# damlobster/DotsBoxesAZ

Measured on AMD Instinct MI355X. Metric: mcts_node_expansions_per_sec, higher is better.
Workload: dtype f32 via f16x3 (hi,lo)-split MFMA, f32 accumulate; max |dp|,|dv| vs torch fp32 = 1e-6 (tests/test_hip_nn.py)

## Files before the change

dotsboxesaz_amd/csrc/nn.hip:

```cpp
#include <math.h>
#include <stddef.h>
#include <stdlib.h>
#include <string.h>

#include <map>
#include <string>
#include <vector>

#include "nn.h"
#include "tower_perm.h"
#include "tower_plan.h"

typedef float f32x4 __attribute__((ext_vector_type(4)));

#define CONV_THREADS 512

struct TowerArgs;
typedef void (*TowerKernel)(Geo, TowerArgs);
struct TowerLaunch {
    TowerKernel kernel;
    size_t lds;
    int role, S;
    enum Grid { PER_GROUP, ONE_ROUND, ONE_ROUND_AT_MOST } grid;
    bool fallback;
// ... 118 lines not shown
#define F16_GUARD 60000.0f

union u128h { f32x4 f; f16x8 h; };

template <int C, int PREC>
__device__ __forceinline__ void act_store(float *lds, int row, int c, float v, bool &ovf)
{
    if constexpr (PREC == 0) {
        lds[row * (C + 8) + c] = v;
    } else {
        _Float16 *h = reinterpret_cast<_Float16 *>(lds) + (size_t)row * ((C + 8) * 2);
        const float x = v * ACT_SCALE;
        ovf |= fabsf(x) > F16_GUARD;
        const _Float16 hi = (_Float16)x;
        h[c] = hi;
        h[C + c] = (_Float16)(x - (float)hi);
    }
}
template <int C, int PREC>
__device__ __forceinline__ float act_load(const float *lds, int row, int c)
{
    if constexpr (PREC == 0) {
        return lds[row * (C + 8) + c];
    } else {
        const _Float16 *h = reinterpret_cast<const _Float16 *>(lds) + (size_t)row * ((C + 8) * 2);
        return ((float)h[c] + (float)h[C + c]) * (1.0f / ACT_SCALE);
    }
}

__device__ __forceinline__ f32x4 relu4(f32x4 v)
{
    v[0] = fmaxf(v[0], 0.f); v[1] = fmaxf(v[1], 0.f); v[2] = fmaxf(v[2], 0.f); v[3] = fmaxf(v[3], 0.f);
    return v;
}
__device__ __forceinline__ float max4(f32x4 v) { return fmaxf(fmaxf(v[0], v[1]), fmaxf(v[2], v[3])); }

template <int C>
__device__ __forceinline__ void h3_store(_Float16 *ph, bool valid, f32x4 v)
{
    union { f16x2 h[2]; u32x2 u; } oh, ol;
#pragma unroll
    for (int q = 0; q < 2; q++) {
        const f32x2 x = {v[2 * q], v[2 * q + 1]};
        const f16x2 h = __builtin_convertvector(x, f16x2);
        oh.h[q] = h;
        ol.h[q] = __builtin_convertvector(x - __builtin_convertvector(h, f32x2), f16x2);
    }
    if (valid) {
        *reinterpret_cast<u32x2 *>(ph) = oh.u;
        *reinterpret_cast<u32x2 *>(ph + C) = ol.u;
    }
}

#ifdef DBAZ_STAMP
#define STAMP(var)                                                                      \
    do {                                                                                \
        __builtin_amdgcn_sched_barrier(0);                                              \
        asm volatile("s_memtime %0\n\ts_waitcnt lgkmcnt(0)" : "=s"(var)::"memory");     \
        __builtin_amdgcn_sched_barrier(0);                                              \
    } while (0)
#else
#define STAMP(var) do { } while (0)
#endif

struct WPre { f32x4 h0, l0, h1, l1; };

template <int C>
__device__ __forceinline__ void wpre_load(WPre &pre, const f32x4 *wpk_layer, int wave, int lane)
{
    constexpr int N = 9 * (C / 32);
    const f32x4 *wb = wpk_layer + (size_t)(wave & 3) * N * 2 * 64 + lane;
    pre.h0 = wb[0];
    pre.l0 = wb[64];
    pre.h1 = wb[128];
    pre.l1 = wb[192];
}

template <int C, int NTT, bool RR = false>
__device__ __forceinline__ void conv_lds_h3(const f32x4 *__restrict__ src4, f32x4 *dst4, const f32x4 *__restrict__ wpk ,
                                            const float *__restrict__ bias, float oscale, const int *vm, int rowbase,
                                            int zbase, int W, int R, int wave, int lane, int residual, bool &ovf_out, int tbase,
                                            const float *post_s, const float *post_t, WPre &pre, const f32x4 *next_wpk,
                                            f32x4 (&res)[NTT], unsigned long long *stamps = nullptr)
{
    static_assert(!RR || C <= 64, "one cout tile per wave");

    unsigned long long t0 = 0, t1 = 0, t2 = 0, t3 = 0;
    (void)t0; (void)t1; (void)t2; (void)t3; (void)stamps;
    constexpr int S4 = (C + 8) / 4;
    constexpr int KS = C / 32;
    constexpr int LO = C / 8;
    constexpr int N = 9 * KS;
    const int jrow = lane & 15, gq = lane >> 4;
    bool ovf = false;
    for (int ct = wave & 3; ct < C / 16; ct += 4) {
        f32x4 acc[NTT];
#pragma unroll
        for (int t = 0; t < NTT; t++) acc[t] = (f32x4){0.f, 0.f, 0.f, 0.f};
        const f32x4 *wbase = wpk + (size_t)ct * N * 2 * 64 + lane;
        u128h a_h[3], a_l[3];
        u128h bh[NTT], bl[NTT];
        const char *sb = reinterpret_cast<const char *>(src4);
        int ab[NTT];
#pragma unroll
        for (int t = 0; t < NTT; t++)
            ab[t] = ((vm[t] & 1) ? rowbase + (-W - 1) * S4 : zbase + ((rowbase + (-W - 1) * S4) & 15) - t * 16 * S4) * 16;
// ... 60 lines not shown
                    rl[t] = *reinterpret_cast<const u32x2 *>(ph + C);
                }
            }
        }
        float vmax = 0.0f;
#pragma unroll
        for (int t = 0; t < NTT; t++) {
            const int row = (tbase + t) * 16 + jrow;
            f32x4 v = acc[t] * oscale + bv;
            if (residual) {
                if constexpr (RR) {
                    v += res[t];
                } else {
                    union { unsigned int u; f16x2 h; } c0, c1, d0, d1;
                    c0.u = rh[t][0]; c1.u = rh[t][1]; d0.u = rl[t][0]; d1.u = rl[t][1];
                    v[0] += (float)c0.h[0] + (float)d0.h[0];
                    v[1] += (float)c0.h[1] + (float)d0.h[1];
                    v[2] += (float)c1.h[0] + (float)d1.h[0];
                    v[3] += (float)c1.h[1] + (float)d1.h[1];
                }
            }
            v = relu4(v);
            if constexpr (RR) {
                if (residual) res[t] = v;
            }
            if (post_s) {
                v = v * *reinterpret_cast<const f32x4 *>(post_s + ct * 16 + gq * 4) +
                    *reinterpret_cast<const f32x4 *>(post_t + ct * 16 + gq * 4);
                vmax = fmaxf(vmax, fmaxf(fmaxf(fabsf(v[0]), fabsf(v[1])), fmaxf(fabsf(v[2]), fabsf(v[3]))));
            } else {
                vmax = fmaxf(vmax, max4(v));
            }
            h3_store<C>(dsth + (size_t)row * (S4 * 8) + ct * 16 + gq * 4, row < R, v);
        }
        ovf |= vmax > F16_GUARD;
        STAMP(t3);
#ifdef DBAZ_STAMP
        if (stamps) { stamps[0] += t1 - t0; stamps[1] += t2 - t1; stamps[2] += t3 - t2; }
#endif
    }
    ovf_out |= ovf;
}

__device__ __forceinline__ void glds16(const void *gsrc, unsigned lds_dst)
{
    unsigned keep;
    asm volatile("s_mov_b32 %0, m0\n\ts_mov_b32 m0, %2\n\ts_nop 0\n\tglobal_load_lds_dwordx4 %1, off\n\ts_mov_b32 m0, %0"
                 : "=&s"(keep) : "v"(gsrc), "s"(lds_dst) : "memory");
}
__device__ __forceinline__ unsigned lds_addr(const void *p)
{
    return (unsigned)(size_t)(const __attribute__((address_space(3))) char *)p;
}
#define PAT_NONE 4
__host__ __device__ constexpr int pat_drop(int pat, int t)
{
    constexpr int top = 0007, bottom = 0700, left = 0111, right = 0444;
    return pat == PAT_NONE || t > 1 ? 0
         : t == 0 ? (pat < 2 ? top : bottom)
                  : (pat == 0 || pat == 3 ? left : right);
}
static_assert(pat_drop(0, 0) == TP_TOP && pat_drop(0, 1) == TP_LEFT && pat_drop(1, 0) == TP_TOP && pat_drop(1, 1) == TP_RIGHT &&
              pat_drop(2, 0) == TP_BOTTOM && pat_drop(2, 1) == TP_RIGHT && pat_drop(3, 0) == TP_BOTTOM && pat_drop(3, 1) == TP_LEFT,
              "the kernel's patterns are those the row table is built and verified for (tower_perm.h)");

template <int C, int NTT, int PAT = PAT_NONE>
__device__ __forceinline__ void conv_lds_h3_c2(const f32x4 *__restrict__ src4, f32x4 *dst4, const f32x4 *__restrict__ wpk ,
                                               const float *__restrict__ bias, float oscale, const int *vm, int rowbase,
                                               int zbase, int W, int R, int wave, int lane, int residual, bool &ovf_out, int tbase,
                                               WPre (&pre)[2], const f32x4 *next_wpk, f32x4 (&res)[2][NTT],
                                               unsigned long long *stamps, f32x4 *wring, const int *rb = nullptr)
{
    constexpr bool PERM = PAT != PAT_NONE;
    static_assert(!PERM || NTT == 4, "the row table is built for 4 tiles per wave pair");
    unsigned long long t0 = 0, t1 = 0, t2 = 0, t3 = 0;
    (void)t0; (void)t1; (void)t2; (void)t3; (void)stamps;
    static_assert(C == 64, "two cout tiles per wave x two wave parities = 64 channels");
    constexpr int S4 = (C + 8) / 4;
    constexpr int KS = C / 32;
    constexpr int LO = C / 8;
    constexpr int N = 9 * KS;
    static_assert(N % 2 == 0, "the next layer's step 0 must land in slot 0");
    const int jrow = lane & 15, gq = lane >> 4;
    const int ct0 = (wave & 1) * 2;
    f32x4 acc[2][NTT];
#pragma unroll
    for (int c = 0; c < 2; c++)
#pragma unroll
        for (int t = 0; t < NTT; t++) acc[c][t] = (f32x4){0.f, 0.f, 0.f, 0.f};
    u128h a_h[2][2], a_l[2][2];
    u128h bh[NTT], bl[NTT];
    const char *sb = reinterpret_cast<const char *>(src4);
    int ab[NTT];
    auto tap_unit = [&](int offr) -> int { return rowbase + offr * S4; };
    auto kept = [](int t, int tap) constexpr -> bool { return !((pat_drop(PAT, t) >> tap) & 1); };
    auto n_kept = [&](int tap) constexpr -> int { int n = 0; for (int t = 0; t < NTT; t++) n += kept(t, tap) ? 1 : 0; return n; };
    auto tile_off = [](int t) constexpr -> int { return PERM ? 0 : t * 256 * S4; };
    auto set_ab = [&](int tap) {
        if constexpr (PERM) {
            int offu = ((tap / 3 - 1) * W + (tap % 3 - 1)) * S4;
            asm volatile("" : "+s"(offu));
#pragma unroll
            for (int t = 0; t < NTT; t++)
                if (kept(t, tap)) {
                    const int un = rb[t] + offu;
                    ab[t] = (((vm[t] >> tap) & 1) ? un : zbase + (un & 15)) * 16;
                }
        } else {
            const int un = tap_unit((tap / 3 - 1) * W + (tap % 3 - 1));
            const int zt = zbase + (un & 15);
#pragma unroll
            for (int t = 0; t < NTT; t++) ab[t] = (((vm[t] >> tap) & 1) ? un : zt - t * 16 * S4) * 16;
        }
    };
    set_ab(0);
    STAMP(t0);
    const f32x4 *dsrc = wpk + ((size_t)(wave >> 1) * N * 2 + (wave & 1)) * 64 + lane;
    const f32x4 *dnext = next_wpk ? next_wpk + ((size_t)(wave >> 1) * N * 2 + (wave & 1)) * 64 + lane : nullptr;
    const f32x4 *rsrc = wring + (size_t)ct0 * 2 * 64 + lane;
    const unsigned ring_dst = __builtin_amdgcn_readfirstlane(lds_addr(wring + (size_t)wave * 64));
#pragma unroll
    for (int c = 0; c < 2; c++) { a_h[c][0].f = pre[c].h0; a_l[c][0].f = pre[c].l0; }
#pragma unroll
    for (int t = 0; t < NTT; t++)
        if (kept(t, 0)) bh[t].f = *reinterpret_cast<const f32x4 *>(sb + ab[t] + tile_off(t));
#pragma unroll
    for (int t = 0; t < NTT; t++)
        if (kept(t, 0)) bl[t].f = *reinterpret_cast<const f32x4 *>(sb + ab[t] + tile_off(t) + LO * 16);
    STAMP(t1);
#pragma unroll
    for (int i = 0; i < N; i++) {
        const int cur = i & 1, nxt = (i + 1) & 1;
        const int tap = i / KS, ni = i + 1, ntap = ni / KS, nks = ni % KS;
        if (i + 2 < N) glds16(dsrc + (size_t)(i + 2) * 128, ring_dst + (i & 1) * (WRING_UNITS * 16));
        else if (dnext) glds16(dnext + (size_t)(i + 2 - N) * 128, ring_dst + (i & 1) * (WRING_UNITS * 16));
        if (ni < N) {
            const f32x4 *r1 = rsrc + (size_t)(ni & 1) * WRING_UNITS;
            a_h[0][nxt].f = r1[0]; a_l[0][nxt].f = r1[64]; a_h[1][nxt].f = r1[128]; a_l[1][nxt].f = r1[192];
        }
        __builtin_amdgcn_sched_barrier(0);
#pragma unroll
        for (int t = 0; t < NTT; t++)
            if (kept(t, tap)) {
                acc[0][t] = __builtin_amdgcn_mfma_f32_16x16x32_f16(a_h[0][cur].h, bh[t].h, acc[0][t], 0, 0, 0);
                acc[1][t] = __builtin_amdgcn_mfma_f32_16x16x32_f16(a_h[1][cur].h, bh[t].h, acc[1][t], 0, 0, 0);
            }
        if (ni < N && nks == 0) set_ab(ntap);
        __builtin_amdgcn_sched_barrier(0);
#pragma unroll
        for (int t = 0; t < NTT; t++) {
            if (kept(t, tap)) {
                acc[0][t] = __builtin_amdgcn_mfma_f32_16x16x32_f16(a_l[0][cur].h, bh[t].h, acc[0][t], 0, 0, 0);
                acc[1][t] = __builtin_amdgcn_mfma_f32_16x16x32_f16(a_l[1][cur].h, bh[t].h, acc[1][t], 0, 0, 0);
            }
            if (ni < N && kept(t, ntap)) bh[t].f = *reinterpret_cast<const f32x4 *>(sb + ab[t] + tile_off(t) + nks * 64);
            __builtin_amdgcn_sched_barrier(0);
        }
#pragma unroll
        for (int t = 0; t < NTT; t++) {
            if (kept(t, tap)) {
                acc[0][t] = __builtin_amdgcn_mfma_f32_16x16x32_f16(a_h[0][cur].h, bl[t].h, acc[0][t], 0, 0, 0);
                acc[1][t] = __builtin_amdgcn_mfma_f32_16x16x32_f16(a_h[1][cur].h, bl[t].h, acc[1][t], 0, 0, 0);
            }
            if (ni < N && kept(t, ntap)) bl[t].f = *reinterpret_cast<const f32x4 *>(sb + ab[t] + tile_off(t) + nks * 64 + LO * 16);
            __builtin_amdgcn_sched_barrier(0);
        }
        if (ni >= N) asm volatile("s_waitcnt vmcnt(0)" ::: "memory");
        else if (n_kept(ntap) == NTT) asm volatile("s_waitcnt vmcnt(0) lgkmcnt(%0)" ::"n"(2 * NTT) : "memory");
        else if (n_kept(ntap) == NTT - 1) asm volatile("s_waitcnt vmcnt(0) lgkmcnt(%0)" ::"n"(2 * NTT - 2) : "memory");
        else if (n_kept(ntap) == NTT - 2) asm volatile("s_waitcnt vmcnt(0) lgkmcnt(%0)" ::"n"(2 * NTT > 4 ? 2 * NTT - 4 : 0) : "memory");
        else asm volatile("s_waitcnt vmcnt(0) lgkmcnt(0)" ::: "memory");
        if (ni < N) __builtin_amdgcn_s_barrier();
        __builtin_amdgcn_sched_barrier(0);
    }
    STAMP(t2);
    f32x4 bv[2];
#pragma unroll
    for (int c = 0; c < 2; c++) {
        bv[c] = *reinterpret_cast<const f32x4 *>(bias + (ct0 + c) * 16 + gq * 4);
        asm volatile("" ::"v"(bv[c]));
    }
    __builtin_amdgcn_sched_barrier(0);
    if (next_wpk) {
        pre[0].h0 = rsrc[0]; pre[0].l0 = rsrc[64]; pre[1].h0 = rsrc[128]; pre[1].l0 = rsrc[192];
    }
    __builtin_amdgcn_sched_barrier(0);
    _Float16 *dsth = reinterpret_cast<_Float16 *>(dst4);
    float vmax = 0.0f;
#pragma unroll
    for (int c = 0; c < 2; c++) {
        const int col = (ct0 + c) * 16 + gq * 4;
#pragma unroll
        for (int t = 0; t < NTT; t++) {
            f32x4 v = acc[c][t] * oscale + bv[c];
            if (residual) v += res[c][t];
            v = relu4(v);
            if (residual) res[c][t] = v;
            vmax = fmaxf(vmax, max4(v));
            if constexpr (PERM) {
                h3_store<C>(dsth + (rb[t] - gq) * 8 + col, vm[t] != 0, v);
            } else {
                const int row = (tbase + t) * 16 + jrow;
                h3_store<C>(dsth + (size_t)row * (S4 * 8) + col, row < R, v);
            }
        }
    }
    ovf_out |= vmax > F16_GUARD;
    STAMP(t3);
#ifdef DBAZ_STAMP
    if (stamps) { stamps[0] += t1 - t0; stamps[1] += t2 - t1; stamps[2] += t3 - t2; }
#endif
}

__device__ __forceinline__ int cut_n(int n, int round, int defer_max)
{
    if (round <= 0) return n;
    const int n_full = (n / round) * round;
    return (n_full > 0 && n - n_full <= defer_max) ? n_full : n;
}

struct TowerArgs {
    const float *feat;
    const int32_t *list;
    const int32_t *n_dev;
    const float *in_s, *in_t;
    const float *w0, *b0;
    const float *tw;
    const float *tb;
    const float *tosc;
    const float *hw, *hb;
    const float *hwp;
    float hosc;
    const float *w0p;
    float osc0;
    unsigned long long *stamp_out;
    const float *wfc, *bfc;
    const float *wv1, *bv1;
    float *P, *V;
    int KP, ntp, ntv, vf, AS;
    int32_t *n_used;
    int *overflow;
    int *ovf_flags;
    int fallback;
    int S, nblocks, hc;
    int role, S_main, S_small, S_mid, S_big, S_huge, cus;
    int cut_round, cut_defer;
    const unsigned char *perm;
};
static_assert(offsetof(TowerArgs, wfc) == 136, "see stamp_out: the fields from wfc on keep these kernel-argument offsets");

__device__ __forceinline__ void head_fc_fused(const Geo &g, const TowerArgs &a, const float *stage, float *lg, int ns, int s0,
                                              int tid, int nthr)
{
    const int lane = tid & 63, wave = tid >> 6, nw = nthr >> 6;
    const int K = a.hc * g.HW, KC = a.KP / 16, NJ = a.ntp + a.ntv, LGS = NJ * 16 + 1, A = g.A;
    const int jrow = lane & 15, gq = lane >> 4;
    const f32x4 *wfc4 = reinterpret_cast<const f32x4 *>(a.wfc);
    const float *rowp = stage + (size_t)min(jrow, ns - 1) * (2 * K) + gq * 4;
    constexpr int G = 8;
    for (int job = wave; job < NJ; job += nw) {
        const float *brow = rowp + (job < a.ntp ? 0 : K);
        const f32x4 *wp = wfc4 + (size_t)job * KC * 64 + lane;
        f32x4 acc = (f32x4){0.f, 0.f, 0.f, 0.f};
// ... 167 lines not shown
            X4[zu + tid] = (f32x4){0.f, 0.f, 0.f, 0.f};
            Y4[zu + tid] = (f32x4){0.f, 0.f, 0.f, 0.f};
        }
    }
    __syncthreads();
    const int jrow = lane & 15, gq = lane >> 4;
    const bool first = wave < 4;
    const int tbase = C2 ? (wave >> 1) * NTA : (first ? 0 : NTA);
    constexpr bool PERMOK = C2 && NTA == 4;
    bool perm_on = false;
    if constexpr (PERMOK) perm_on = a.perm != nullptr;
    int vm[NTA];
    int rb[NTA];
    int rrow[NTA];
    (void)rb; (void)rrow;
#pragma unroll
    for (int t = 0; t < NTA; t++) {
        int row = (tbase + t) * 16 + jrow;
        if constexpr (PERMOK) {
            if (perm_on) row = a.perm[row];
            rb[t] = row * S4 + gq;
            rrow[t] = min(row, R - 1);
        }
        int pos = row % HW, y = pos / W, x = pos - y * W;
        int m = 0;
#pragma unroll
        for (int tap = 0; tap < 9; tap++) {
            int yy = y + tap / 3 - 1, xx = x + tap % 3 - 1;
            m |= ((yy >= 0) && (yy < H) && (xx >= 0) && (xx < W)) ? (1 << tap) : 0;
        }
        vm[t] = row < R ? m : 0;
    }
    const int rowbase = (tbase * 16 + jrow) * S4 + gq;
    const int zbase = zu;
    if constexpr (PREC == 0) {
        const size_t wl = (size_t)C * C * 9;
        for (int l = 0; l < 2 * a.nblocks; l++) {
            const f32x4 *src = (l & 1) ? Y4 : X4;
            f32x4 *dst = (l & 1) ? X4 : Y4;
            if (first) conv_lds_f32<C, NTA>(src, dst, a.tw + (size_t)l * wl, a.tb + l * C, vm, rowbase, zbase, W, R, wave, lane, l & 1, tbase);
            else if constexpr (NTB > 0) conv_lds_f32<C, NTB>(src, dst, a.tw + (size_t)l * wl, a.tb + l * C, vm, rowbase, zbase, W, R, wave, lane, l & 1, tbase);
            __syncthreads();
        }
    } else {
        const f32x4 *tw4 = reinterpret_cast<const f32x4 *>(a.tw);
        const size_t wl = (size_t)C * C * 9 * 2 * 2 / 16;
        const int NL = 2 * a.nblocks;
        WPre pre;
        WPre pre2[2];
        (void)pre2;
        if constexpr (!C2) {
            if (NL > 0) wpre_load<C>(pre, tw4, wave, lane);
        }
        unsigned long long stamps[4] = {0, 0, 0, 0};
        unsigned long long tb0 = 0, tb1 = 0, tk0 = 0, tk1 = 0;
        (void)tb0; (void)tb1; (void)tk0; (void)tk1;
        f32x4 res[2][NTA];
        (void)res;
        if constexpr (RR || C2) {
            const _Float16 *xh = reinterpret_cast<const _Float16 *>(X4);
#pragma unroll
            for (int c = 0; c < (C2 ? 2 : 1); c++) {
                const int col = (C2 ? (wave & 1) * 2 + c : wave & 3) * 16 + gq * 4;
                if (col < C) {
#pragma unroll
                    for (int t = 0; t < NTA; t++) {
                        int row = min((tbase + t) * 16 + jrow, R - 1);
                        if constexpr (PERMOK) row = rrow[t];
                        const _Float16 *ph = xh + (size_t)row * (S4 * 8) + col;
#pragma unroll
                        for (int e = 0; e < 4; e++) res[c][t][e] = (float)ph[e] + (float)ph[C + e];
                    }
                }
            }
        }
        f32x4 *wring = nullptr;
        if constexpr (C2) {
            wring = Y4 + img_units;
            if (NL > 0) {
                const f32x4 *d0 = tw4 + ((size_t)(wave >> 1) * (9 * (C / 32)) * 2 + (wave & 1)) * 64 + lane;
                const unsigned dst = __builtin_amdgcn_readfirstlane(lds_addr(wring + (size_t)wave * 64));
                glds16(d0, dst);
                glds16(d0 + 128, dst + WRING_UNITS * 16);
                asm volatile("s_waitcnt vmcnt(0)" ::: "memory");
            }
            __syncthreads();
            {
                const f32x4 *r0 = wring + (size_t)((wave & 1) * 2) * 2 * 64 + lane;
                pre2[0].h0 = r0[0]; pre2[0].l0 = r0[64]; pre2[1].h0 = r0[128]; pre2[1].l0 = r0[192];
                asm volatile("s_waitcnt lgkmcnt(0)" ::: "memory");
            }
            __syncthreads();
        }
        STAMP(tk0);
        tL0 = tk0;
        const int pat = perm_on ? __builtin_amdgcn_readfirstlane(wave >> 1) : PAT_NONE;
        (void)pat;
        for (int l = 0; l < NL; l++) {
            const f32x4 *src = (l & 1) ? Y4 : X4;
            f32x4 *dst = (l & 1) ? X4 : Y4;
            const f32x4 *nxt = l + 1 < NL ? tw4 + (size_t)(l + 1) * wl : nullptr;
            if constexpr (PERMOK) {
#define C2_PAT(P) conv_lds_h3_c2<C, NTA, P>(src, dst, tw4 + (size_t)l * wl, a.tb + l * C, a.tosc[l], vm, rowbase, zbase, W, R, wave, lane, l & 1, ovf, tbase, pre2, nxt, res, stamps, wring, rb)
                switch (pat) {
                case 0: C2_PAT(0); break;
                case 1: C2_PAT(1); break;
                case 2: C2_PAT(2); break;
                case 3: C2_PAT(3); break;
                default: C2_PAT(PAT_NONE); break;
                }
#undef C2_PAT
            } else if constexpr (C2) {
                conv_lds_h3_c2<C, NTA>(src, dst, tw4 + (size_t)l * wl, a.tb + l * C, a.tosc[l], vm, rowbase, zbase, W, R, wave, lane, l & 1, ovf, tbase, pre2, nxt, res, stamps, wring);
            } else {
                if (first) conv_lds_h3<C, NTA, RR>(src, dst, tw4 + (size_t)l * wl, a.tb + l * C, a.tosc[l], vm, rowbase, zbase, W, R, wave, lane, l & 1, ovf, tbase, nullptr, nullptr, pre, nxt, res[0], stamps);
                else if constexpr (NTB > 0) conv_lds_h3<C, NTB, RR>(src, dst, tw4 + (size_t)l * wl, a.tb + l * C, a.tosc[l], vm, rowbase, zbase, W, R, wave, lane, l & 1, ovf, tbase, nullptr, nullptr, pre, nxt, reinterpret_cast<f32x4(&)[NTB]>(res[0]), stamps);
            }
            STAMP(tb0);
            __syncthreads();
            STAMP(tb1);
#ifdef DBAZ_STAMP
            stamps[3] += tb1 - tb0;
#endif
        }
#ifdef DBAZ_STAMP
        STAMP(tk1);
        tL1 = tk1;
        if (a.stamp_out && lane == 0) {
            unsigned long long *o = a.stamp_out + ((size_t)blockIdx.x * 8 + wave) * 10;
            o[0] = stamps[0]; o[1] = stamps[1]; o[2] = stamps[2]; o[3] = stamps[3]; o[4] = tk1 - tk0;
        }
#endif
    }
    bool heads_done = false;
    if constexpr (PREC == 1) {
        if (a.hwp) {
            constexpr int KS = C / 32, LO = C / 8;
            const int OC = 2 * a.hc, n_ct = ((OC + 15) & ~15) / 16, ngrp = (NTHR >> 6) / n_ct;
            const int ct = wave % n_ct, grp = wave / n_ct;
            const int NT = (R + 15) / 16;
            float *stage = Y;
            const f32x4 *wp = reinterpret_cast<const f32x4 *>(a.hwp) + (size_t)ct * KS * 2 * 64 + lane;
            u128h ah[KS], al[KS];
#pragma unroll
            for (int ks = 0; ks < KS; ks++) { ah[ks].f = wp[(size_t)ks * 128]; al[ks].f = wp[(size_t)ks * 128 + 64]; }
            const int hj = lane & 15, hq = lane >> 4;
            const int oc0 = ct * 16 + hq * 4;
            f32x4 bv = (f32x4){0.f, 0.f, 0.f, 0.f};
#pragma unroll
            for (int r = 0; r < 4; r++) if (oc0 + r < OC) bv[r] = a.hb[oc0 + r];
            for (int t = grp; t < NT; t += ngrp) {
                const int row = t * 16 + hj;
                const int rr = min(row, R - 1);
                const f32x4 *bp = X4 + (size_t)rr * S4 + hq;
                f32x4 acc = (f32x4){0.f, 0.f, 0.f, 0.f};
#pragma unroll
                for (int ks = 0; ks < KS; ks++) {
                    u128h bh, bl;
                    bh.f = bp[ks * 4];
                    bl.f = bp[ks * 4 + LO];
                    acc = __builtin_amdgcn_mfma_f32_16x16x32_f16(ah[ks].h, bh.h, acc, 0, 0, 0);
                    acc = __builtin_amdgcn_mfma_f32_16x16x32_f16(al[ks].h, bh.h, acc, 0, 0, 0);
                    acc = __builtin_amdgcn_mfma_f32_16x16x32_f16(ah[ks].h, bl.h, acc, 0, 0, 0);
                }
                if (row < R) {
                    const int sidx = row / HW, pp = row - sidx * HW;
                    const f32x4 v = acc * a.hosc + bv;
#pragma unroll
                    for (int r = 0; r < 4; r++)
                        if (oc0 + r < OC) stage[(sidx * OC + oc0 + r) * HW + pp] = fmaxf(v[r], 0.0f);
                }
            }
            if (tid < 16) stage[(size_t)ns * OC * HW + tid] = 0.0f;
            __syncthreads();
            head_fc_fused(g, a, stage, stage + (size_t)S * OC * HW + 16, ns, s0, tid, NTHR);
            heads_done = true;
        }
    }
    if (!heads_done) {
        const int OC = 2 * a.hc;
        float *wl = Y;
        float *stage = Y + OC * (C + 4);
        for (int i = tid; i < OC * C; i += NTHR) {
            int o = i / C, c = i - o * C;
            wl[o * (C + 4) + c] = a.hw[i];
        }
        __syncthreads();
        if (tid < R) {
            const int row = tid;
            float xr[C];
#pragma unroll
            for (int c = 0; c < C; c++) xr[c] = act_load<C, PREC>(X, row, c);
            const int sidx = row / HW, p = row - sidx * HW;
            for (int oc = 0; oc < OC; oc++) {
                float acc = a.hb[oc];
                const float *wr = wl + oc * (C + 4);
#pragma unroll
                for (int c = 0; c < C; c += 4) {
                    const f32x4 w4 = *reinterpret_cast<const f32x4 *>(wr + c);
                    acc += xr[c] * w4[0] + xr[c + 1] * w4[1] + xr[c + 2] * w4[2] + xr[c + 3] * w4[3];
                }
                stage[(sidx * OC + oc) * HW + p] = fmaxf(acc, 0.0f);
            }
        }
        if (tid < 16) stage[(size_t)ns * OC * HW + tid] = 0.0f;
        __syncthreads();
        head_fc_fused(g, a, stage, stage + (size_t)S * OC * HW + 16, ns, s0, tid, NTHR);
    }
    if (PREC == 1 && ovf) {
        for (int i = 0; i < ns; i++) a.ovf_flags[s0 + i] = 1;
        atomicOr(a.overflow, 1);
    }
#ifdef DBAZ_STAMP
    STAMP(tE1);
    if (PREC == 1 && a.stamp_out && lane == 0) {
        unsigned long long *o = a.stamp_out + ((size_t)blockIdx.x * 8 + wave) * 10;
        o[5] = tL0 - tE0;
        o[6] = tE1 - tL1;
        o[7] = tE1 - tE0;
        o[8] = __builtin_amdgcn_s_memrealtime() - tR0;
    }
#endif
}

__device__ __forceinline__ int tower_split(const TowerArgs &a, int n, int &n_full)
{
    return tower_split(a.cus, a.S_main, a.S_small, a.S_mid, a.S_big, a.S_huge, n, n_full);
}

template <int C, int NTA, int NTB, int PREC, bool C2 = false>
__global__ void __launch_bounds__(CONV_THREADS, 1) k_tower(Geo g, TowerArgs a)
{
    extern __shared__ __attribute__((aligned(16))) float lds[];
    const int n = cut_n(*a.n_dev, a.cut_round, a.cut_defer);
    const int S = a.S;
    int first_sample = 0, limit = n;
    {
        int n_full;
        const int mode = tower_split(a, n, n_full);
        if (a.role == 0) {
            if (mode) limit = n_full;
        } else {
            if (mode != a.role) return;
            first_sample = n_full;
        }
    }
    if constexpr (PREC == 0) {
        if (a.fallback) {
            __shared__ int n_redo;
            __shared__ int redo_grp[CONV_THREADS];
            if (threadIdx.x == 0) n_redo = 0;
            __syncthreads();
            {
                const int gt = blockIdx.x + threadIdx.x * gridDim.x;
                const long long st = (long long)gt * S;
                if (st < n) {
                    int any = 0;
                    const int m = min(S, n - (int)st);
                    for (int i = 0; i < m; i++) any |= a.ovf_flags[st + i];
                    if (any) {
                        for (int i = 0; i < m; i++) a.ovf_flags[st + i] = 0;
                        redo_grp[atomicAdd(&n_redo, 1)] = gt;
                        atomicAdd(a.overflow + 1, m);
                    }
                }
            }
            __syncthreads();
            const int nr = n_redo;
            for (int r = 0; r < nr; r++) {
// ... 669 lines not shown
        std::vector<double> si, ti;
        if (!bn_affine(nn, "bn_input", 3, si, ti, err)) return DBAZ_EINVAL;
        std::vector<float> fs(si.begin(), si.end()), ft(ti.begin(), ti.end());
        nn->in_s = nn_upload(nn, fs);
        nn->in_t = nn_upload(nn, ft);
    }
    {
        auto w = sd_get(nn, "resnet.conv0.weight", (size_t)Cr * 27, err); if (!w) return DBAZ_EINVAL;
        auto b = sd_get(nn, "resnet.conv0.bias", Cr, err); if (!b) return DBAZ_EINVAL;
        std::vector<double> sc, tc;
        if (!bn_affine(nn, "resnet.bn0", Cr, sc, tc, err)) return DBAZ_EINVAL;
        std::vector<float> pk((size_t)27 * C, 0.0f), bias(C, 0.0f);
        for (int co = 0; co < Cr; co++) {
            for (int ci = 0; ci < 3; ci++)
                for (int tap = 0; tap < 9; tap++)
                    pk[(size_t)(tap * 3 + ci) * C + co] = (float)((double)(*w)[((size_t)co * 3 + ci) * 9 + tap] * sc[co]);
            bias[co] = (float)((double)(*b)[co] * sc[co] + tc[co]);
        }
        nn->w0 = nn_upload(nn, pk);
        nn->b0 = nn_upload(nn, bias);
        nn->w0p = nullptr;
        if (nn->precision == 1 && C >= 32) {
            int sw;
            nn->w0p = nn_upload(nn, pack_h3(C, 32, C, 27, [&](int co, int k) { return (double)pk[(size_t)k * C + co]; }, sw));
            nn->osc0 = (float)ldexp(1.0, -sw);
        }
    }
    {
        std::vector<float> pk_all, bias_all, pk32_all, bias32_all;
        const bool both = nn->precision == 1 && C >= 32;
        nn->osc_host.clear();
        for (int i = 0; i < nn->blocks; i++) {
            std::string p = "resnet.resblocks." + std::to_string(i);
            if (!pack_conv(nn, p + ".conv1", p + ".bn1", C, pk_all, bias_all, err, true, both ? &pk32_all : nullptr, both ? &bias32_all : nullptr)) return DBAZ_EINVAL;
            if (!pack_conv(nn, p + ".conv2", p + ".bn2", C, pk_all, bias_all, err, true, both ? &pk32_all : nullptr, both ? &bias32_all : nullptr)) return DBAZ_EINVAL;
        }
        nn->tw = nn_upload(nn, pk_all);
        nn->tb = nn_upload(nn, bias_all);
        nn->tw32 = nn->tb32 = nullptr;
        nn->ovf_flags = nullptr;
        if (both) {
            nn->tw32 = nn_upload(nn, pk32_all);
            nn->tb32 = nn_upload(nn, bias32_all);
            nn->ovf_flags = nn_alloc<int>(nn, (size_t)nn->max_batch + 16);
            if (!nn->tw32 || !nn->tb32 || !nn->ovf_flags) { err = "hipMalloc failed (f32 fallback weights)"; return DBAZ_EDEVICE; }
            (void)hipMemset(nn->ovf_flags, 0, ((size_t)nn->max_batch + 16) * sizeof(int));
        }
        if (nn->osc_host.empty()) nn->osc_host.push_back(1.0f);
        nn->tosc = nn_upload(nn, nn->osc_host);
        nn->overflow = nn_alloc<int>(nn, 4);
        if (!nn->tw || !nn->tb || !nn->tosc || !nn->overflow) { err = "hipMalloc failed (tower weights)"; return DBAZ_EDEVICE; }
        (void)hipMemset(nn->overflow, 0, 16);
#ifdef DBAZ_STAMP
        nn->stamp_out = nn_alloc<unsigned long long>(nn, (size_t)nn->max_batch * 8 * 10);
        (void)hipMemset(nn->stamp_out, 0, (size_t)nn->max_batch * 8 * 10 * 8);
#endif
    }
    {
        std::vector<float> hw((size_t)2 * hc * C, 0.0f), hb(2 * hc);
        const char *heads[2] = {"policy_head", "value_head"};
        for (int h = 0; h < 2; h++) {
            std::string p = heads[h];
            auto w = sd_get(nn, p + ".conv0.weight", (size_t)hc * Cr, err); if (!w) return DBAZ_EINVAL;
            auto b = sd_get(nn, p + ".conv0.bias", hc, err); if (!b) return DBAZ_EINVAL;
            std::vector<double> sc, tc;
            if (!bn_affine(nn, p + ".bn0", hc, sc, tc, err)) return DBAZ_EINVAL;
            for (int o = 0; o < hc; o++) {
                for (int c = 0; c < Cr; c++) hw[(size_t)(h * hc + o) * C + c] = (float)((double)(*w)[(size_t)o * Cr + c] * sc[o]);
                hb[h * hc + o] = (float)((double)(*b)[o] * sc[o] + tc[o]);
            }
        }
        nn->hw = nn_upload(nn, hw);
        nn->hb = nn_upload(nn, hb);
        nn->hwp = nullptr;
        const int OCP = (2 * hc + 15) & ~15, n_ct = OCP / 16;
        if (nn->precision == 1 && C >= 32 && (n_ct == 1 || n_ct == 2 || n_ct == 4 || n_ct == 8)) {
            int sw;
            nn->hwp = nn_upload(nn, pack_h3(OCP, C, 2 * hc, C, [&](int oc, int ci) { return (double)hw[(size_t)oc * C + ci]; }, sw));
            nn->hosc = (float)ldexp(1.0, -(sw + ACT_SHIFT));
        }
    }
    {
        auto wp = sd_get(nn, "policy_head.fc.weight", (size_t)A * K, err); if (!wp) return DBAZ_EINVAL;
        auto bp = sd_get(nn, "policy_head.fc.bias", A, err); if (!bp) return DBAZ_EINVAL;
        auto w0 = sd_get(nn, "value_head.fc0.weight", (size_t)vf * K, err); if (!w0) return DBAZ_EINVAL;
        auto b0 = sd_get(nn, "value_head.fc0.bias", vf, err); if (!b0) return DBAZ_EINVAL;
        auto w1 = sd_get(nn, "value_head.fc1.weight", vf, err); if (!w1) return DBAZ_EINVAL;
        auto b1 = sd_get(nn, "value_head.fc1.bias", 1, err); if (!b1) return DBAZ_EINVAL;
        const int KP = (K + 15) & ~15, ntp = (A + 15) / 16, ntv = (vf + 15) / 16, NJ = ntp + ntv;
        if (NJ >= 32) { err = "head FC tile does not fit LDS"; return DBAZ_EINVAL; }
        std::vector<float> bias((size_t)NJ * 16, 0.0f);
        for (int o = 0; o < A; o++) bias[o] = (*bp)[o];
        for (int o = 0; o < vf; o++) bias[ntp * 16 + o] = (*b0)[o];
        nn->wfc = nn_upload(nn, pack_fc(NJ, KP, K, [&](int o) -> const float * {
            if (o < ntp * 16) return o < A ? wp->data() + (size_t)o * K : nullptr;
            return o - ntp * 16 < vf ? w0->data() + (size_t)(o - ntp * 16) * K : nullptr;
        }));
        nn->bfc = nn_upload(nn, bias);
        nn->wv1 = nn_upload(nn, *w1);
        nn->bv1 = nn_upload(nn, *b1);
        nn->KP = KP; nn->ntp = ntp; nn->ntv = ntv;
    }
    if (!nn->wfc || !nn->wv1 || !nn->w0) { err = "hipMalloc failed (network buffers)"; return DBAZ_EDEVICE; }
    TowerPlan &tp = nn->plan;
    if (const char *why = tower_plan_build(g.H, g.W, C, hc, vf, nn->precision, tp)) { err = why; return DBAZ_EINVAL; }
    {
        int dev = 0, cus = 0;
        if (hipGetDevice(&dev) == hipSuccess && hipDeviceGetAttribute(&cus, hipDeviceAttributeMultiprocessorCount, dev) == hipSuccess && cus > 0)
            nn->cus = cus;
    }
    nn->tperm = nullptr;
    if (tp.c2 && tp.NT_c2 == 4) {
        int tab[TOWER_PERM_ROWS];
        if (tower_perm_build(g.H, g.W, tp.S_c2, tab) > 0) {
            nn->tperm = nn_upload(nn, std::vector<unsigned char>(tab, tab + TOWER_PERM_ROWS));
            if (!nn->tperm) { err = "hipMalloc failed (row table)"; return DBAZ_EDEVICE; }
        }
    }
    std::vector<TowerLaunch> &L = nn->launches;
    L.clear();
    if (tp.c2) L.push_back({tower_kernel_c2(tp.NT_c2), tp.conv_lds_c2, 0, tp.S_main(), TowerLaunch::PER_GROUP, false});
    else L.push_back({tower_kernel(C, tp.NTT, nn->precision), tp.conv_lds, 0, tp.S_main(), TowerLaunch::PER_GROUP, false});
    if (tp.use_rem) {
        L.push_back({tower_kernel_rem(C, tp.c2 != 0), tp.conv_lds, -1, tp.S_main(), TowerLaunch::ONE_ROUND, false});
    } else {
        const int tail_S[3] = {tp.S_small, tp.S_mid, tp.S_big}, tail_ntt[3] = {2, 4, 5};
        for (int i = 0; i < 3; i++)
            if (tail_S[i] > 0) L.push_back({tower_kernel(C, tail_ntt[i], nn->precision), tp.conv_lds, i + 1, tail_S[i], TowerLaunch::ONE_ROUND, false});
    }
    if (nn->tw32) L.push_back({tower_kernel(C, tp.NTT, 0), tp.conv_lds, 0, tp.S, TowerLaunch::ONE_ROUND_AT_MOST, true});
    hipError_t he = hipSuccess;
    for (const TowerLaunch &l : L) {
        if (!l.kernel) { err = "no tower kernel for this geometry"; return DBAZ_EINVAL; }
        if (he == hipSuccess) he = hipFuncSetAttribute((const void *)l.kernel, hipFuncAttributeMaxDynamicSharedMemorySize, (int)l.lds);
    }
    if (he != hipSuccess) {
        (void)hipGetLastError();
        err = std::string("hipFuncSetAttribute: ") + hipGetErrorString(he);
        return DBAZ_EDEVICE;
    }
    nn->ready = true;
    return DBAZ_OK;
}

void nn_forward(NNState *nn, hipStream_t s, const float *feat, const int32_t *list_dev, const int32_t *n_dev, int max_n,
                float *P, float *V, int AS, hipEvent_t ev_begin, hipEvent_t ev_end, int cut_round, int cut_defer, int32_t *n_used)
{
    const Geo &g = nn->g;
    const int hc = nn->hc;
    if (max_n > nn->max_batch) max_n = nn->max_batch;
    if (nn->kind == DBAZ_EVAL_SIMPLENN) {
        SimpleArgs sa;
        sa.feat = feat; sa.list = list_dev; sa.n_dev = n_dev; sa.w0 = nn->w0; sa.b0 = nn->b0; sa.s0 = nn->sn_s0; sa.t0 = nn->sn_t0;
        sa.tw = nn->tw; sa.tb = nn->tb; sa.ts = nn->sn_ts; sa.tt = nn->sn_tt; sa.tosc = nn->tosc; sa.flat = nn->sn_flat;
        sa.overflow = nn->overflow; sa.S = nn->sn_S;
        if (ev_begin) (void)hipEventRecord(ev_begin, s);
        const int grid = (max_n + nn->sn_S - 1) / nn->sn_S;
        if (nn->precision == 1) hipLaunchKernelGGL(k_simple_trunk<1>, dim3(grid), dim3(CONV_THREADS), nn->sn_lds, s, g, sa);
        else hipLaunchKernelGGL(k_simple_trunk<0>, dim3(grid), dim3(CONV_THREADS), nn->sn_lds, s, g, sa);
        if (ev_end) (void)hipEventRecord(ev_end, s);
        DenseArgs d0;
        d0.n_dev = n_dev; d0.in = nn->sn_flat; d0.w = nn->sn_w0; d0.b = nn->sn_b0; d0.ps = nn->sn_ps0; d0.pt = nn->sn_pt0;
        d0.out = nn->sn_h1; d0.K = 1024; d0.O = 512; d0.RS4 = dense_rs4(1024); d0.dup = 0;
        hipLaunchKernelGGL(k_dense, dim3((max_n + 15) / 16), dim3(256), (size_t)16 * d0.RS4 * 16, s, d0);
        DenseArgs d1;
        d1.n_dev = n_dev; d1.in = nn->sn_h1; d1.w = nn->sn_w1; d1.b = nn->sn_b1; d1.ps = nn->sn_ps1; d1.pt = nn->sn_pt1;
        d1.out = nn->hact; d1.K = 512; d1.O = 256; d1.RS4 = dense_rs4(512); d1.dup = 1;
        hipLaunchKernelGGL(k_dense, dim3((max_n + 15) / 16), dim3(256), (size_t)16 * d1.RS4 * 16, s, d1);
        HeadArgs ha;
        ha.list = list_dev; ha.n_dev = n_dev; ha.hact = nn->hact; ha.wfc = nn->wfc; ha.bfc = nn->bfc;
        ha.P = P; ha.V = V; ha.K = 256; ha.KP = 256; ha.ntp = nn->ntp; ha.ntv = nn->ntv; ha.AS = AS;
        hipLaunchKernelGGL(k_head_fc, dim3((max_n + 16 * HEAD_MT - 1) / (16 * HEAD_MT)), dim3(256), nn->fc_lds, s, g, ha);
        return;
    }
    TowerArgs ta;
    ta.feat = feat; ta.list = list_dev; ta.n_dev = n_dev; ta.in_s = nn->in_s; ta.in_t = nn->in_t; ta.w0 = nn->w0; ta.b0 = nn->b0;
    ta.tw = nn->tw; ta.tb = nn->tb; ta.tosc = nn->tosc; ta.hw = nn->hw; ta.hb = nn->hb; ta.hwp = nn->hwp; ta.hosc = nn->hosc; ta.w0p = nn->w0p; ta.osc0 = nn->osc0;
    ta.overflow = nn->overflow; ta.ovf_flags = nn->ovf_flags; ta.nblocks = nn->blocks; ta.hc = hc;
    ta.wfc = nn->wfc; ta.bfc = nn->bfc; ta.wv1 = nn->wv1; ta.bv1 = nn->bv1; ta.P = P; ta.V = V; ta.KP = nn->KP; ta.ntp = nn->ntp;
    ta.ntv = nn->ntv; ta.vf = nn->vf; ta.AS = AS; ta.n_used = n_used;
    ta.stamp_out = nn->stamp_out;
    if (ev_begin) (void)hipEventRecord(ev_begin, s);
    const TowerPlan &tp = nn->plan;
    ta.S_main = tp.S_main(); ta.S_small = tp.S_small; ta.S_mid = tp.S_mid; ta.S_big = tp.S_big; ta.S_huge = tp.S_huge();
    ta.cus = nn->cus; ta.cut_round = cut_round; ta.cut_defer = cut_defer;
    ta.perm = tp.c2 ? nn->tperm : nullptr;
    for (const TowerLaunch &l : nn->launches) {
        ta.role = l.role; ta.S = l.S; ta.fallback = l.fallback;
        if (l.fallback) {
            ta.S_main = l.S; ta.S_small = ta.S_mid = ta.S_big = ta.S_huge = 0;
            ta.tw = nn->tw32; ta.tb = nn->tb32; ta.w0p = nullptr; ta.hwp = nullptr;
        }
        const int groups = (max_n + l.S - 1) / l.S;
        const int grid = l.grid == TowerLaunch::PER_GROUP ? groups : l.grid == TowerLaunch::ONE_ROUND ? nn->cus : std::min(groups, nn->cus);
        hipLaunchKernelGGL(l.kernel, dim3(grid), dim3(CONV_THREADS), l.lds, s, g, ta);
    }
    if (ev_end) (void)hipEventRecord(ev_end, s);
}

void nn_round_info(const NNState *nn, int *round, int *rem_max)
{
    *round = 0; *rem_max = 0;
    if (!nn || nn->kind != DBAZ_EVAL_RESNET) return;
    const TowerPlan &tp = nn->plan;
    *round = nn->cus * tp.S_main();
    const int s_rem = tp.c2 ? tp.S : std::max(tp.S_big, std::max(tp.S_mid, tp.S_small));
    *rem_max = nn->cus * s_rem;
}

double nn_flops_per_sample(const NNState *nn)
{
    const Geo &g = nn->g;
    if (nn->kind == DBAZ_EVAL_SIMPLENN)
        return 2.0 * (16 * 27 * 256 + 3.0 * 16 * 2304 * 256 + 4 * 2304 * 256 + 1024 * 512 + 512 * 256 + 256 * 33);
    const double HW = g.HW, C = nn->Craw, hc = nn->hc, K = hc * HW;
    double f = 2.0 * HW * 27 * C + 2.0 * nn->blocks * 2.0 * HW * 9 * C * C;
    f += 2.0 * 2.0 * HW * C * hc + 2.0 * K * g.A + 2.0 * K * nn->vf + 2.0 * nn->vf;
    return f;
}

int nn_read_stamps(NNState *nn, unsigned long long *out, int n_wg)
{
    if (!nn || !nn->stamp_out) return -1;
    return (int)hipMemcpy(out, nn->stamp_out, (size_t)n_wg * 8 * 10 * 8, hipMemcpyDeviceToHost);
}

int nn_overflowed(NNState *nn)
{
    if (!nn || !nn->overflow || nn->tw32) return 0;
    int v = 0;
    (void)hipMemcpy(&v, nn->overflow, 4, hipMemcpyDeviceToHost);
    return v;
}

long long nn_fallback_evals(NNState *nn)
{
    if (!nn || !nn->overflow || !nn->tw32) return 0;
    int v[2] = {0, 0};
    (void)hipMemcpy(v, nn->overflow, 8, hipMemcpyDeviceToHost);
    return v[1];
}
```

Measured before the change: 4.750 million.

## Deepen conv weight DMA ring to three slots in the dst activation buffer

For the c2 conv bodies with 3 or 4 tiles per wave pair, the weight prefetch ring moves from two slots to DBAZ_RING_P (default 3). The extra slots are placed in the destination activation buffer, and the per-step wait becomes vmcnt(NS-2) instead of vmcnt(0), so global-to-LDS weight loads have more steps to land before they are consumed. The next layer's first two steps still go to the original ring. Stamp instrumentation is also widened to record DMA-wait and barrier time. The risk is that the ring region aliases the output image before it is written, and there is more address arithmetic per step.

```diff
diff --git a/dotsboxesaz_amd/csrc/nn.hip b/dotsboxesaz_amd/csrc/nn.hip
--- a/dotsboxesaz_amd/csrc/nn.hip
+++ b/dotsboxesaz_amd/csrc/nn.hip
@@ -194,6 +194,7 @@
     }
 }
 
+#define STAMP_WORDS 16
 #ifdef DBAZ_STAMP
 #define STAMP(var)                                                                      \
     do {                                                                                \
@@ -360,6 +361,25 @@
 {
     return (unsigned)(size_t)(const __attribute__((address_space(3))) char *)p;
 }
+template <int VM, int LG>
+__device__ __forceinline__ void wait_vm_lgkm()
+{
+    if constexpr (LG < 0) asm volatile("s_waitcnt vmcnt(%0)" ::"n"(VM) : "memory");
+    else asm volatile("s_waitcnt vmcnt(%0) lgkmcnt(%1)" ::"n"(VM), "n"(LG) : "memory");
+}
+template <int LG>
+__device__ __forceinline__ void wait_step(int vm)
+{
+    switch (vm) {
+    case 0: wait_vm_lgkm<0, LG>(); break;
+    case 1: wait_vm_lgkm<1, LG>(); break;
+    case 2: wait_vm_lgkm<2, LG>(); break;
+    case 3: wait_vm_lgkm<3, LG>(); break;
+    case 4: wait_vm_lgkm<4, LG>(); break;
+    case 5: wait_vm_lgkm<5, LG>(); break;
+    default: wait_vm_lgkm<6, LG>(); break;
+    }
+}
 #define PAT_NONE 4
 __host__ __device__ constexpr int pat_drop(int pat, int t)
 {
@@ -371,6 +391,20 @@
 static_assert(pat_drop(0, 0) == TP_TOP && pat_drop(0, 1) == TP_LEFT && pat_drop(1, 0) == TP_TOP && pat_drop(1, 1) == TP_RIGHT &&
               pat_drop(2, 0) == TP_BOTTOM && pat_drop(2, 1) == TP_RIGHT && pat_drop(3, 0) == TP_BOTTOM && pat_drop(3, 1) == TP_LEFT,
               "the kernel's patterns are those the row table is built and verified for (tower_perm.h)");
+
+#ifndef DBAZ_RING_P
+#define DBAZ_RING_P 3
+#endif
+static_assert(DBAZ_RING_P >= 2 && DBAZ_RING_P <= 8, "prefetch distance");
+__host__ __device__ constexpr int wring_deep_slots(int ntt)
+{
+    const int units = (64 * (ntt - 1) + 1) * ((64 + 8) / 4);
+    int p = DBAZ_RING_P;
+    while (p > 2 && p * WRING_UNITS > units) p--;
+    return p > 2 ? p : 0;
+}
+static_assert(DBAZ_RING_P != 3 || (wring_deep_slots(4) == 3 && wring_deep_slots(3) == 3 && wring_deep_slots(2) == 0 && wring_deep_slots(1) == 0),
+              "4 and 3 tiles per wave pair hold the three slots, the smaller bodies keep the two-slot ring");
 
 template <int C, int NTT, int PAT = PAT_NONE>
 __device__ __forceinline__ void conv_lds_h3_c2(const f32x4 *__restrict__ src4, f32x4 *dst4, const f32x4 *__restrict__ wpk ,
@@ -381,9 +415,12 @@
 {
     constexpr bool PERM = PAT != PAT_NONE;
     static_assert(!PERM || NTT == 4, "the row table is built for 4 tiles per wave pair");
-    unsigned long long t0 = 0, t1 = 0, t2 = 0, t3 = 0;
-    (void)t0; (void)t1; (void)t2; (void)t3; (void)stamps;
+    unsigned long long t0 = 0, t1 = 0, t2 = 0, t3 = 0, ua = 0, uc = 0, ud = 0;
+    (void)t0; (void)t1; (void)t2; (void)t3; (void)ua; (void)uc; (void)ud; (void)stamps;
+    unsigned w_dma = 0, w_bar = 0, w_cal = 0;
+    (void)w_dma; (void)w_bar; (void)w_cal;
     static_assert(C == 64, "two cout tiles per wave x two wave parities = 64 channels");
+    constexpr int NS = wring_deep_slots(NTT);
     constexpr int S4 = (C + 8) / 4;
     constexpr int KS = C / 32;
     constexpr int LO = C / 8;
@@ -422,11 +459,21 @@
         }
     };
     set_ab(0);
+    STAMP(ua);
     STAMP(t0);
+#ifdef DBAZ_STAMP
+    w_cal = (unsigned)(t0 - ua);
+#endif
     const f32x4 *dsrc = wpk + ((size_t)(wave >> 1) * N * 2 + (wave & 1)) * 64 + lane;
     const f32x4 *dnext = next_wpk ? next_wpk + ((size_t)(wave >> 1) * N * 2 + (wave & 1)) * 64 + lane : nullptr;
     const f32x4 *rsrc = wring + (size_t)ct0 * 2 * 64 + lane;
     const unsigned ring_dst = __builtin_amdgcn_readfirstlane(lds_addr(wring + (size_t)wave * 64));
+    const f32x4 *dnx = (next_wpk ? next_wpk : wpk) + ((size_t)(wave >> 1) * N * 2 + (wave & 1)) * 64 + lane;
+    const f32x4 *rsrc_i = dst4 + (size_t)ct0 * 2 * 64 + lane;
+    const unsigned ring_dst_i = __builtin_amdgcn_readfirstlane(lds_addr(dst4 + (size_t)wave * 64));
+    (void)dnx; (void)rsrc_i; (void)ring_dst_i; (void)dnext;
+    static_assert(NS == 0 || (NS >= 3 && N - NS >= 1 && NS * WRING_UNITS <= (64 * (NTT - 1) + 1) * S4),
+                  "the slots end inside the rows every workgroup of this body has; the next layer's steps 0 and 1 are issued from step 1 on");
 #pragma unroll
     for (int c = 0; c < 2; c++) { a_h[c][0].f = pre[c].h0; a_l[c][0].f = pre[c].l0; }
 #pragma unroll
@@ -440,10 +487,18 @@
     for (int i = 0; i < N; i++) {
         const int cur = i & 1, nxt = (i + 1) & 1;
         const int tap = i / KS, ni = i + 1, ntap = ni / KS, nks = ni % KS;
-        if (i + 2 < N) glds16(dsrc + (size_t)(i + 2) * 128, ring_dst + (i & 1) * (WRING_UNITS * 16));
-        else if (dnext) glds16(dnext + (size_t)(i + 2 - N) * 128, ring_dst + (i & 1) * (WRING_UNITS * 16));
+        if constexpr (NS == 0) {
+            if (i + 2 < N) glds16(dsrc + (size_t)(i + 2) * 128, ring_dst + (i & 1) * (WRING_UNITS * 16));
+            else if (dnext) glds16(dnext + (size_t)(i + 2 - N) * 128, ring_dst + (i & 1) * (WRING_UNITS * 16));
+        } else {
+            if (i == 0)
+#pragma unroll
+                for (int j = 2; j < NS; j++) glds16(dsrc + (size_t)j * 128, ring_dst_i + j * (WRING_UNITS * 16));
+            if (i + NS < N) glds16(dsrc + (size_t)(i + NS) * 128, ring_dst_i + (i % NS) * (WRING_UNITS * 16));
+            else if (i + NS - N < 2) glds16(dnx + (size_t)(i + NS - N) * 128, ring_dst + (i + NS - N) * (WRING_UNITS * 16));
+        }
         if (ni < N) {
-            const f32x4 *r1 = rsrc + (size_t)(ni & 1) * WRING_UNITS;
+            const f32x4 *r1 = NS > 0 && ni >= 2 ? rsrc_i + (size_t)(ni % NS) * WRING_UNITS : rsrc + (size_t)(ni & 1) * WRING_UNITS;
             a_h[0][nxt].f = r1[0]; a_l[0][nxt].f = r1[64]; a_h[1][nxt].f = r1[128]; a_l[1][nxt].f = r1[192];
         }
         __builtin_amdgcn_sched_barrier(0);
@@ -473,13 +528,29 @@
             if (ni < N && kept(t, ntap)) bl[t].f = *reinterpret_cast<const f32x4 *>(sb + ab[t] + tile_off(t) + nks * 64 + LO * 16);
             __builtin_amdgcn_sched_barrier(0);
         }
-        if (ni >= N) asm volatile("s_waitcnt vmcnt(0)" ::: "memory");
-        else if (n_kept(ntap) == NTT) asm volatile("s_waitcnt vmcnt(0) lgkmcnt(%0)" ::"n"(2 * NTT) : "memory");
-        else if (n_kept(ntap) == NTT - 1) asm volatile("s_waitcnt vmcnt(0) lgkmcnt(%0)" ::"n"(2 * NTT - 2) : "memory");
-        else if (n_kept(ntap) == NTT - 2) asm volatile("s_waitcnt vmcnt(0) lgkmcnt(%0)" ::"n"(2 * NTT > 4 ? 2 * NTT - 4 : 0) : "memory");
-        else asm volatile("s_waitcnt vmcnt(0) lgkmcnt(0)" ::: "memory");
+        STAMP(ua);
+        if constexpr (NS == 0) {
+            if (ni >= N) asm volatile("s_waitcnt vmcnt(0)" ::: "memory");
+            else if (n_kept(ntap) == NTT) asm volatile("s_waitcnt vmcnt(0) lgkmcnt(%0)" ::"n"(2 * NTT) : "memory");
+            else if (n_kept(ntap) == NTT - 1) asm volatile("s_waitcnt vmcnt(0) lgkmcnt(%0)" ::"n"(2 * NTT - 2) : "memory");
+            else if (n_kept(ntap) == NTT - 2) asm volatile("s_waitcnt vmcnt(0) lgkmcnt(%0)" ::"n"(2 * NTT > 4 ? 2 * NTT - 4 : 0) : "memory");
+            else asm volatile("s_waitcnt vmcnt(0) lgkmcnt(0)" ::: "memory");
+        } else {
+            const int vmw = NS - 2 < N - 1 - i ? NS - 2 : N - 1 - i;
+            if (ni >= N) wait_step<-1>(vmw);
+            else if (n_kept(ntap) == NTT) wait_step<2 * NTT>(vmw);
+            else if (n_kept(ntap) == NTT - 1) wait_step<2 * NTT - 2>(vmw);
+            else if (n_kept(ntap) == NTT - 2) wait_step<(2 * NTT > 4 ? 2 * NTT - 4 : 0)>(vmw);
+            else wait_step<0>(vmw);
+        }
+        STAMP(uc);
         if (ni < N) __builtin_amdgcn_s_barrier();
         __builtin_amdgcn_sched_barrier(0);
+        STAMP(ud);
+#ifdef DBAZ_STAMP
+        w_dma += (unsigned)(uc - ua);
+        if (ni < N) w_bar += (unsigned)(ud - uc);
+#endif
     }
     STAMP(t2);
     f32x4 bv[2];
@@ -516,7 +587,7 @@
     ovf_out |= vmax > F16_GUARD;
     STAMP(t3);
 #ifdef DBAZ_STAMP
-    if (stamps) { stamps[0] += t1 - t0; stamps[1] += t2 - t1; stamps[2] += t3 - t2; }
+    if (stamps) { stamps[0] += t1 - t0; stamps[1] += t2 - t1; stamps[2] += t3 - t2; stamps[4] += w_dma; stamps[5] += w_bar; stamps[6] += w_cal; }
 #endif
 }
 
@@ -790,7 +861,7 @@
         if constexpr (!C2) {
             if (NL > 0) wpre_load<C>(pre, tw4, wave, lane);
         }
-        unsigned long long stamps[4] = {0, 0, 0, 0};
+        unsigned long long stamps[7] = {0, 0, 0, 0, 0, 0, 0};
         unsigned long long tb0 = 0, tb1 = 0, tk0 = 0, tk1 = 0;
         (void)tb0; (void)tb1; (void)tk0; (void)tk1;
         f32x4 res[2][NTA];
@@ -865,8 +936,9 @@
         STAMP(tk1);
         tL1 = tk1;
         if (a.stamp_out && lane == 0) {
-            unsigned long long *o = a.stamp_out + ((size_t)blockIdx.x * 8 + wave) * 10;
+            unsigned long long *o = a.stamp_out + ((size_t)blockIdx.x * 8 + wave) * STAMP_WORDS;
             o[0] = stamps[0]; o[1] = stamps[1]; o[2] = stamps[2]; o[3] = stamps[3]; o[4] = tk1 - tk0;
+            o[10] = stamps[4]; o[11] = stamps[5]; o[12] = stamps[6];
         }
 #endif
     }
@@ -952,7 +1024,7 @@
 #ifdef DBAZ_STAMP
     STAMP(tE1);
     if (PREC == 1 && a.stamp_out && lane == 0) {
-        unsigned long long *o = a.stamp_out + ((size_t)blockIdx.x * 8 + wave) * 10;
+        unsigned long long *o = a.stamp_out + ((size_t)blockIdx.x * 8 + wave) * STAMP_WORDS;
         o[5] = tL0 - tE0;
         o[6] = tE1 - tL1;
         o[7] = tE1 - tE0;
@@ -1728,8 +1800,8 @@
         if (!nn->tw || !nn->tb || !nn->tosc || !nn->overflow) { err = "hipMalloc failed (tower weights)"; return DBAZ_EDEVICE; }
         (void)hipMemset(nn->overflow, 0, 16);
 #ifdef DBAZ_STAMP
-        nn->stamp_out = nn_alloc<unsigned long long>(nn, (size_t)nn->max_batch * 8 * 10);
-        (void)hipMemset(nn->stamp_out, 0, (size_t)nn->max_batch * 8 * 10 * 8);
+        nn->stamp_out = nn_alloc<unsigned long long>(nn, (size_t)nn->max_batch * 8 * STAMP_WORDS);
+        (void)hipMemset(nn->stamp_out, 0, (size_t)nn->max_batch * 8 * STAMP_WORDS * 8);
 #endif
     }
     {
@@ -1795,6 +1867,10 @@
     }
     std::vector<TowerLaunch> &L = nn->launches;
     L.clear();
+    if (tp.c2 && (size_t)wring_deep_slots(tp.NT_c2) * WRING_UNITS > (size_t)tp.S_c2 * g.HW * ((C + 8) / 4)) {
+        err = "the weight ring does not fit the activation image";
+        return DBAZ_EINVAL;
+    }
     if (tp.c2) L.push_back({tower_kernel_c2(tp.NT_c2), tp.conv_lds_c2, 0, tp.S_main(), TowerLaunch::PER_GROUP, false});
     else L.push_back({tower_kernel(C, tp.NTT, nn->precision), tp.conv_lds, 0, tp.S_main(), TowerLaunch::PER_GROUP, false});
     if (tp.use_rem) {
@@ -1898,7 +1974,7 @@
 int nn_read_stamps(NNState *nn, unsigned long long *out, int n_wg)
 {
     if (!nn || !nn->stamp_out) return -1;
-    return (int)hipMemcpy(out, nn->stamp_out, (size_t)n_wg * 8 * 10 * 8, hipMemcpyDeviceToHost);
+    return (int)hipMemcpy(out, nn->stamp_out, (size_t)n_wg * 8 * STAMP_WORDS * 8, hipMemcpyDeviceToHost);
 }
 
 int nn_overflowed(NNState *nn)
```

Result: faster. 4.831 million, median of 6 (+1.7%).
